# Vandermode/ELD

Measured on AMD Instinct MI355X. Metric: raw megapixels/sec (noise-synth + U-Net step), higher is better.
Workload: dtype f32; 1 GPU; BASELINE.json configs[1]: full ELD noise model (PGRU, SonyA7S2 params) on 4x1424x2128 packed raw + U-Net fp32 train step (fwd, L1, bwd, Adam), 8 frames per GPU; images_per_gpu=8, global_batch=8, parallelism=dp1

## Files before the change

eld_amd/csrc/conv_wgrad.hip:

```cpp
#include <stdlib.h>
#include "conv.h"

#define TW 32
#define JB 32

typedef __bf16 bf16x8 __attribute__((ext_vector_type(8)));
typedef short s16x4 __attribute__((ext_vector_type(4)));
typedef int i32x4_t __attribute__((ext_vector_type(4)));
typedef _Float16 half8 __attribute__((ext_vector_type(8)));

enum { ALG_F32 = 0, ALG_BFM = 1, ALG_X3 = 2, ALG_H2 = 3 };

template <typename T, int MODE, int WCO, int TH, int ALG>
__global__ __launch_bounds__(256, 2) void wgrad_kernel(const WgradArgs a) {
    constexpr bool BFM = ALG == ALG_BFM, X3 = ALG == ALG_X3, H2 = ALG == ALG_H2;
    static_assert(!(X3 || H2) || sizeof(T) == 4, "x3 / h2: fp32 inputs");
    constexpr int ES = sizeof(T);
    constexpr int EPU = 16 / ES;
    constexpr int LES = X3 ? 6 : (BFM ? 2 : 4);
    constexpr int TAPS = MODE == CONV_3X3 ? 9 : 4;
    constexpr int WPIX = 4 / WCO;
    constexpr int COB = 32 * WCO;
    constexpr int TPIX = TH * TW;
    constexpr int PW = TPIX / WPIX;
// ... 237 lines not shown
        for (int s_ = 0; s_ < KS; ++s_) {
            const int cur = s_ & 1;
            if (s_ + 1 < KS) read_step(s_ + 1, fa[cur ^ 1], fb[cur ^ 1]);
            __builtin_amdgcn_sched_barrier(0);
            bsum += fa[cur];
#pragma unroll
            for (int t = 0; t < TAPS; ++t) acc[t] = __builtin_amdgcn_mfma_f32_32x32x2f32(fa[cur], fb[cur][t], acc[t], 0, 0, 0);
            __builtin_amdgcn_sched_barrier(0);
        }
        }
    }

    __syncthreads();
    float* red = lds;
    const size_t pbase = (size_t)ps * TAPS * a.CA * a.CBp;
#pragma unroll
    for (int t = 0; t < TAPS; ++t) {
        if (WPIX > 1) {
            if (wpix > 0) {
#pragma unroll
                for (int i = 0; i < 16; ++i) red[(((wpix - 1) * WCO + wco) * 16 + i) * 64 + lane] = acc[t][i];
            }
            __syncthreads();
            if (wpix == 0) {
                for (int w = 0; w < WPIX - 1; ++w)
#pragma unroll
                    for (int i = 0; i < 16; ++i) acc[t][i] += red[((w * WCO + wco) * 16 + i) * 64 + lane];
            }
            __syncthreads();
        }
        if (wpix == 0) {
#pragma unroll
            for (int i = 0; i < 16; ++i) {
                const int row = (i & 3) + 8 * (i >> 2) + 4 * hi;
                a.part[pbase + ((size_t)t * a.CA + i0 + wco * 32 + row) * a.CBp + j0 + m] = H2 ? acc[t][i] * (1.0f / sc_g) * (1.0f / sc_x) : acc[t][i];
            }
        }
    }
    if (a.bpart && jb == 0) {
        red[wave * 64 + lane] = bsum;
        __syncthreads();
        if (tid < COB) {
            const int wc = tid / 32, mm = tid % 32;
            float s = 0.f;
            for (int wp = 0; wp < WPIX; ++wp) s += red[(wp * WCO + wc) * 64 + mm] + red[(wp * WCO + wc) * 64 + 32 + mm];
            a.bpart[(size_t)ps * a.CA + i0 + tid] = H2 ? s * (1.0f / sc_g) : s;
        }
    }
    if constexpr (XSUM) {
        if (xsum_on) {
            __syncthreads();
            float* r = lds;
#pragma unroll
            for (int e = 0; e < EPU; ++e) r[tid * EPU + e] = xs[e];
            __syncthreads();
            if (tid < JB) {
                constexpr int PARTS = JB / EPU;
                const int part = tid / EPU, comp = tid % EPU;
                float s = 0.f;
                for (int k = 0; k < 256 / PARTS; ++k) s += r[(k * PARTS + part) * EPU + comp];
                a.xbpart[(size_t)ps * a.CBp + j0 + tid] = s;
            }
        }
    }
}

template <typename T, int WCO, int WCI, int WPIX, int TH, int TWT, int STREAM = 0>
__global__ __launch_bounds__(512, 2) void wgrad8_kernel(const WgradArgs a) {
    constexpr int ES = sizeof(T), EPU = 16 / ES, NPC = ES == 4 ? 3 : 1, XQ = 32 / EPU;
    static_assert(WCO * WCI * WPIX == 8, "8 waves");
    constexpr int THREADS = 512, TAPS = 9;
    constexpr int COB = 32 * WCO, JBK = 32 * WCI, TPIX = TH * TWT, PW = TPIX / WPIX, KSB = PW / 16;
    static_assert(TWT == 8 || TWT == 16 || TWT == 32, "tile width");
    static_assert(PW % 16 == 0 && PW >= 16, "a wave's pixel slice is a whole number of 16-pixel k-steps");
    constexpr int X_PIX = (TH + 2) * (TWT + 2);
    constexpr int GBLK = TPIX * 32 + (ES == 4 ? 32 : 0);
    constexpr int GPL = GBLK * WCO, XPL = X_PIX * JBK;
    constexpr int G_Q = COB / EPU, G_UNITS = TPIX * G_Q, G_IT = G_UNITS / THREADS;
    static_assert(G_UNITS % THREADS == 0 && THREADS % G_Q == 0, "a thread stages the same channel quad of G in every iteration");
    constexpr int X_UNITS1 = X_PIX * XQ, X_IT = (X_UNITS1 + THREADS - 1) / THREADS;
    extern __shared__ __attribute__((aligned(16))) float lds[];
    bf16_t* ldsG = reinterpret_cast<bf16_t*>(lds);
    bf16_t* ldsX = ldsG + NPC * GPL;

    const int tid = threadIdx.x, lane = tid & 63, wave = tid >> 6;
    const int m = lane & 31, hi = lane >> 5;
    const int wco = wave % WCO, wci = (wave / WCO) % WCI, wpix = wave / (WCO * WCI);
    const int IB = a.CA / COB, JBn = a.CBp / JBK;
    int bid = xcd_block(a.xcd);
    const int jb = bid % JBn; bid /= JBn;
    const int ib = bid % IB;
    const int ps = bid / IB;
    const int i0 = ib * COB, j0 = jb * JBK;
    const bool do_bias = a.bpart != nullptr && jb == 0;

    f32x16 acc[TAPS];
#pragma unroll
    for (int t = 0; t < TAPS; ++t)
#pragma unroll
        for (int i = 0; i < 16; ++i) acc[t][i] = 0.f;
    float4 bsum4 = make_float4(0.f, 0.f, 0.f, 0.f), bsum4b = make_float4(0.f, 0.f, 0.f, 0.f);

    const int ntiles = a.tiles_x * a.tiles_y;
    const int VP = a.vp;
    const bool seam = VP % TH != 0;
    constexpr unsigned OOB = 0xFFFFFFF0u;
    constexpr int G_STEP = THREADS / G_Q;
    const int g_part = tid % G_Q, g_lp0 = tid / G_Q;
    const int g_px0 = g_lp0 % TWT, g_py0 = g_lp0 / TWT;
    const unsigned g_off0 = (unsigned)(g_px0 * a.CA + i0 + g_part * EPU) * (unsigned)ES;
    const int g_lds0 = ((g_part * EPU) >> 5) * GBLK + g_lp0 * 32 + ((g_part * EPU) & 31);
    auto g_pxy = [&](int it, int& dpx, int& dpy) {
        if (G_STEP >= TWT) { dpx = 0; dpy = it * (G_STEP / TWT); }
        else { dpx = (it * G_STEP) % TWT; dpy = (it * G_STEP) / TWT; }
    };
    const int x_part = (int)((unsigned)tid % (unsigned)XQ);
    int x_hyx[X_IT];
#pragma unroll
    for (int it = 0; it < X_IT; ++it) {
        const int hp = (int)((unsigned)(tid + it * THREADS) / (unsigned)XQ);
        const int hy = hp / (TWT + 2);
        x_hyx[it] = (hy << 8) | (hp - hy * (TWT + 2));
    }
    auto x_alive = [&](int it) { return (it + 1) * THREADS <= X_UNITS1 || (int)((unsigned)(tid + it * THREADS) / (unsigned)XQ) < X_PIX; };
    const char* xs[WCI]; int xC[WCI], xc0[WCI];
#pragma unroll
    for (int cb = 0; cb < WCI; ++cb) {
        const int c = j0 + cb * 32;
        if (c < a.C0) { xs[cb] = static_cast<const char*>(a.x0); xC[cb] = a.C0; xc0[cb] = c; }
        else if (c < a.C0 + a.C1) { xs[cb] = static_cast<const char*>(a.x1); xC[cb] = a.C1; xc0[cb] = c - a.C0; }
        else { xs[cb] = nullptr; xC[cb] = 32; xc0[cb] = 0; }
    }
    float4 rg[G_IT], rx[WCI][X_IT];
    const size_t g_img = (size_t)a.H * a.W * a.CA * ES;
    const unsigned g_rowc = (unsigned)(g_py0 * a.W * a.CA) * (unsigned)ES;
    auto load_tile = [&](int tile) {
        int ty, tx;
        band_tile(tile, a.tiles_x, a.tiles_y, a.band, ty, tx);
        const int v0 = ty * TH, x0 = tx * TWT;
        const int img0 = v0 / VP, vrel = v0 - img0 * VP;
        const int wrem = a.W - x0;
        if (!seam || VP - vrel > TH) {
            const __amdgpu_buffer_rsrc_t rs_g = __builtin_amdgcn_make_buffer_rsrc((void*)(static_cast<const char*>(a.g) + (size_t)img0 * g_img), 0, (int)g_img, 0x00020000);
            const int gbase = (vrel * a.W + x0) * a.CA * ES;
#pragma unroll
            for (int it = 0; it < G_IT; ++it) {
                int dpx, dpy;
                g_pxy(it, dpx, dpy);
                const unsigned off = g_off0 + g_rowc + (unsigned)((dpy * a.W + dpx) * a.CA) * (unsigned)ES;
                rg[it] = __builtin_bit_cast(float4, __builtin_amdgcn_raw_buffer_load_b128(rs_g, g_px0 + dpx < wrem ? (int)off : (int)OOB, gbase, 0));
            }
#pragma unroll
            for (int cb = 0; cb < WCI; ++cb) {
                const size_t x_img = (size_t)a.H * a.W * xC[cb] * ES;
                const __amdgpu_buffer_rsrc_t rs_x = __builtin_amdgcn_make_buffer_rsrc((void*)(xs[cb] ? xs[cb] + (size_t)img0 * x_img : nullptr), 0, xs[cb] ? (int)x_img : 0, 0x00020000);
#pragma unroll
                for (int it = 0; it < X_IT; ++it) {
                    const int gy = vrel - 1 + (x_hyx[it] >> 8), gx = x0 - 1 + (x_hyx[it] & 255);
                    const bool ok = x_alive(it) && (unsigned)gy < (unsigned)a.H && (unsigned)gx < (unsigned)a.W;
                    const unsigned off = ok ? (unsigned)((gy * a.W + gx) * xC[cb] + xc0[cb] + x_part * EPU) * (unsigned)ES : OOB;
                    rx[cb][it] = __builtin_bit_cast(float4, __builtin_amdgcn_raw_buffer_load_b128(rs_x, (int)off, 0, 0));
                }
            }
            return;
        }
        const int nimg = a.N - img0 < 2 ? a.N - img0 : 2;
        const int lim0 = a.H - vrel, nxt = VP - vrel;
        const __amdgpu_buffer_rsrc_t rs_g = __builtin_amdgcn_make_buffer_rsrc((void*)(static_cast<const char*>(a.g) + (size_t)img0 * g_img), 0, (int)(g_img * nimg), 0x00020000);
        const unsigned gb0 = (unsigned)((vrel * a.W + x0) * a.CA) * (unsigned)ES;
        const unsigned gb1 = (unsigned)(((a.H - nxt) * a.W + x0) * a.CA) * (unsigned)ES;
#pragma unroll
        for (int it = 0; it < G_IT; ++it) {
            int dpx, dpy;
            g_pxy(it, dpx, dpy);
            const int r = g_py0 + dpy;
            const bool second = r >= nxt;
            const bool ok = (r < lim0 || (second && r - nxt < a.H)) && g_px0 + dpx < wrem;
            const unsigned off = (second ? gb1 : gb0) + g_off0 + g_rowc + (unsigned)((dpy * a.W + dpx) * a.CA) * (unsigned)ES;
            rg[it] = __builtin_bit_cast(float4, __builtin_amdgcn_raw_buffer_load_b128(rs_g, ok ? (int)off : (int)OOB, 0, 0));
        }
#pragma unroll
        for (int cb = 0; cb < WCI; ++cb) {
            const size_t x_img = (size_t)a.H * a.W * xC[cb] * ES;
            const __amdgpu_buffer_rsrc_t rs_x = __builtin_amdgcn_make_buffer_rsrc((void*)(xs[cb] ? xs[cb] + (size_t)img0 * x_img : nullptr), 0, xs[cb] ? (int)(x_img * nimg) : 0, 0x00020000);
#pragma unroll
            for (int it = 0; it < X_IT; ++it) {
                const int r = (x_hyx[it] >> 8) - 1, gx = x0 - 1 + (x_hyx[it] & 255);
                const bool second = r >= nxt;
                const int wrow = second ? a.H + r - nxt : vrel + r;
                const bool rok = second ? r - nxt < a.H : (unsigned)(vrel + r) < (unsigned)a.H;
                const bool ok = x_alive(it) && rok && (unsigned)gx < (unsigned)a.W;
                const unsigned off = ok ? (unsigned)((wrow * a.W + gx) * xC[cb] + xc0[cb] + x_part * EPU) * (unsigned)ES : OOB;
                rx[cb][it] = __builtin_bit_cast(float4, __builtin_amdgcn_raw_buffer_load_b128(rs_x, (int)off, 0, 0));
            }
        }
    };
    auto put3 = [&](bf16_t* d, int plane_elems, const float4& raw) {
        if constexpr (ES == 2) { *reinterpret_cast<float4*>(d) = raw; return; }
        const unsigned x0 = __float_as_uint(raw.x), x1 = __float_as_uint(raw.y), x2 = __float_as_uint(raw.z), x3 = __float_as_uint(raw.w);
        const float r0 = raw.x - __uint_as_float(x0 & 0xFFFF0000u), r1 = raw.y - __uint_as_float(x1 & 0xFFFF0000u);
        const float r2 = raw.z - __uint_as_float(x2 & 0xFFFF0000u), r3 = raw.w - __uint_as_float(x3 & 0xFFFF0000u);
        const unsigned y0 = __float_as_uint(r0), y1 = __float_as_uint(r1), y2 = __float_as_uint(r2), y3 = __float_as_uint(r3);
        const unsigned z0 = __float_as_uint(r0 - __uint_as_float(y0 & 0xFFFF0000u)), z1 = __float_as_uint(r1 - __uint_as_float(y1 & 0xFFFF0000u));
        const unsigned z2 = __float_as_uint(r2 - __uint_as_float(y2 & 0xFFFF0000u)), z3 = __float_as_uint(r3 - __uint_as_float(y3 & 0xFFFF0000u));
        auto hp = [](unsigned lo, unsigned hi_) { return __builtin_amdgcn_perm(hi_, lo, 0x07060302u); };
        *reinterpret_cast<uint2*>(d) = make_uint2(hp(x0, x1), hp(x2, x3));
        *reinterpret_cast<uint2*>(d + plane_elems) = make_uint2(hp(y0, y1), hp(y2, y3));
        *reinterpret_cast<uint2*>(d + 2 * plane_elems) = make_uint2(hp(z0, z1), hp(z2, z3));
    };
    auto store_tile = [&]() {
#pragma unroll
        for (int it = 0; it < G_IT; ++it) {
            put3(ldsG + g_lds0 + it * G_STEP * 32, GPL, rg[it]);
            if (do_bias) {
                if constexpr (ES == 4) { bsum4.x += rg[it].x; bsum4.y += rg[it].y; bsum4.z += rg[it].z; bsum4.w += rg[it].w; }
                else {
                    const uint4 q = __builtin_bit_cast(uint4, rg[it]);
                    const float4 lo = unpack_bf4(make_uint2(q.x, q.y)), hi4 = unpack_bf4(make_uint2(q.z, q.w));
                    bsum4.x += lo.x; bsum4.y += lo.y; bsum4.z += lo.z; bsum4.w += lo.w;
                    bsum4b.x += hi4.x; bsum4b.y += hi4.y; bsum4b.z += hi4.z; bsum4b.w += hi4.w;
                }
            }
        }
#pragma unroll
        for (int cb = 0; cb < WCI; ++cb)
#pragma unroll
            for (int it = 0; it < X_IT; ++it)
                if (x_alive(it)) put3(ldsX + (cb * X_PIX + (int)((unsigned)(tid + it * THREADS) / (unsigned)XQ)) * 32 + x_part * EPU, XPL, rx[cb][it]);
    };

    const int gi = lane & 15, gg = lane >> 4;
    constexpr bool ROWSHARE = STREAM == 2;
    static_assert(!ROWSHARE || (NPC == 3 && TWT == 8 && WPIX == 1 && TH % 2 == 0), "row-shared fragments: fp32, 8-pixel-wide tiles, one pixel slice");
    constexpr int HS = TH / 2;
    const int lq0 = ROWSHARE ? HS * TWT * hi + (gi >> 2) : wpix * PW + 8 * hi + (gi >> 2);
    const int pyq = lq0 / TWT, pxq = lq0 - pyq * TWT;
    const bf16_t* gq = ldsG + wco * GBLK + lq0 * 32 + (gg & 1) * 16 + (gi & 3) * 4;
    const bf16_t* xq = ldsX + (wci * X_PIX + pyq * (TWT + 2) + pxq) * 32 + (gg & 1) * 16 + (gi & 3) * 4;
    auto tr8 = [](const bf16_t* p0) {
        const s16x4 lo = __builtin_amdgcn_ds_read_tr16_b64_v4i16((__attribute__((address_space(3))) s16x4*)p0);
        const s16x4 hi4 = __builtin_amdgcn_ds_read_tr16_b64_v4i16((__attribute__((address_space(3))) s16x4*)(p0 + 4 * 32));
        return __builtin_bit_cast(bf16x8, __builtin_shufflevector(lo, hi4, 0, 1, 2, 3, 4, 5, 6, 7));
    };

    if (ps < ntiles) load_tile(ps);
    for (int tile = ps; tile < ntiles; tile += a.psplit) {
        __syncthreads();
        store_tile();
        __syncthreads();
        if (tile + a.psplit < ntiles) load_tile(tile + a.psplit);
        if constexpr (ROWSHARE) {
            constexpr int GI[6] = {0, 1, 2, 0, 1, 0};
            constexpr int XI[6] = {2, 1, 0, 1, 0, 0};
            constexpr int NU = (HS + 2) * 3;
            bf16x8 gr[3][3], xf[2][3];
            auto readG = [&](int s_, bf16x8 (&g3)[3]) {
#pragma unroll
                for (int pc = 0; pc < 3; ++pc) g3[pc] = tr8(gq + pc * GPL + s_ * TWT * 32);
            };
            auto readF = [&](int a_, int kx, bf16x8 (&x3)[3]) {
#pragma unroll
                for (int pc = 0; pc < 3; ++pc) x3[pc] = tr8(xq + pc * XPL + (a_ * (TWT + 2) + kx) * 32);
            };
            readG(0, gr[0]);
            readF(0, 0, xf[0]);
#pragma unroll
            for (int u = 0; u < NU; ++u) {
                const int a_ = u / 3, kx = u % 3;
                if (u + 1 < NU) readF((u + 1) / 3, (u + 1) % 3, xf[(u + 1) & 1]);
                __builtin_amdgcn_sched_barrier(0);
#pragma unroll
                for (int ky = 2; ky >= 0; --ky) {
                    const int s_ = a_ - ky;
                    if (s_ >= 0 && s_ < HS) {
#pragma unroll
                        for (int q = 0; q < 6; ++q)
                            acc[3 * ky + kx] = __builtin_amdgcn_mfma_f32_32x32x16_bf16(gr[s_ % 3][GI[q]], xf[u & 1][XI[q]], acc[3 * ky + kx], 0, 0, 0);
                    }
                    if (ky == 2 && kx == 2 && a_ + 1 < HS) {
                        __builtin_amdgcn_sched_barrier(0);
                        readG(a_ + 1, gr[(a_ + 1) % 3]);
                    }
                }
                __builtin_amdgcn_sched_barrier(0);
            }
        } else
        if constexpr (NPC == 3 && STREAM == 1) {
            constexpr int GI[6] = {0, 1, 2, 0, 1, 0};
            constexpr int XI[6] = {2, 1, 0, 1, 0, 0};
            constexpr int NBLK = KSB * TAPS;
            bf16x8 ga[2][3], xb[2][3];
            auto readG = [&](int ks, bf16x8 (&g3)[3]) {
#pragma unroll
                for (int pc = 0; pc < 3; ++pc) g3[pc] = tr8(gq + pc * GPL + ks * 16 * 32);
            };
            auto readX = [&](int ks, int t, bf16x8 (&x3)[3]) {
                const int lrel = ks * 16, dy0 = lrel / TWT, dxp = lrel - dy0 * TWT;
                const int xoff = (dy0 + t / 3) * (TWT + 2) + dxp + t % 3;
#pragma unroll
                for (int pc = 0; pc < 3; ++pc) x3[pc] = tr8(xq + pc * XPL + xoff * 32);
            };
            readG(0, ga[0]);
            readX(0, 0, xb[0]);
#pragma unroll
            for (int b = 0; b < NBLK; ++b) {
                const int ks = b / TAPS, t = b % TAPS;
                if (b + 1 < NBLK) {
                    const int ks1 = (b + 1) / TAPS, t1 = (b + 1) % TAPS;
                    readX(ks1, t1, xb[(b + 1) & 1]);
                    if (ks1 != ks) readG(ks1, ga[ks1 & 1]);
                }
                __builtin_amdgcn_sched_barrier(0);
#pragma unroll
                for (int q = 0; q < 6; ++q) acc[t] = __builtin_amdgcn_mfma_f32_32x32x16_bf16(ga[ks & 1][GI[q]], xb[b & 1][XI[q]], acc[t], 0, 0, 0);
                __builtin_amdgcn_sched_barrier(0);
            }
        } else
#pragma unroll
        for (int ks = 0; ks < KSB; ++ks) {
            const int lrel = ks * 16;
            const int dy0 = lrel / TWT, dxp = lrel - dy0 * TWT;
            bf16x8 ga[NPC];
#pragma unroll
            for (int pc = 0; pc < NPC; ++pc) ga[pc] = tr8(gq + pc * GPL + lrel * 32);
#pragma unroll
            for (int t0 = 0; t0 < TAPS; t0 += 3) {
                bf16x8 xb[3][NPC];
#pragma unroll
                for (int tt = 0; tt < 3; ++tt) {
                    const int xoff = (dy0 + t0 / 3) * (TWT + 2) + dxp + tt;
#pragma unroll
                    for (int pc = 0; pc < NPC; ++pc) xb[tt][pc] = tr8(xq + pc * XPL + xoff * 32);
                }
                if constexpr (NPC == 3) {
                    constexpr int GI[6] = {0, 1, 2, 0, 1, 0};
                    constexpr int XI[6] = {2, 1, 0, 1, 0, 0};
#pragma unroll
                    for (int q = 0; q < 6; ++q)
#pragma unroll
                        for (int tt = 0; tt < 3; ++tt)
                            acc[t0 + tt] = __builtin_amdgcn_mfma_f32_32x32x16_bf16(ga[GI[q]], xb[tt][XI[q]], acc[t0 + tt], 0, 0, 0);
                } else {
#pragma unroll
                    for (int tt = 0; tt < 3; ++tt) acc[t0 + tt] = __builtin_amdgcn_mfma_f32_32x32x16_bf16(ga[0], xb[tt][0], acc[t0 + tt], 0, 0, 0);
                }
                __builtin_amdgcn_sched_barrier(0);
            }
        }
    }

    __syncthreads();
    float* red = lds;
    const size_t pbase = (size_t)ps * TAPS * a.CA * a.CBp;
    const int wt = wci * WCO + wco;
#pragma unroll
    for (int t = 0; t < TAPS; ++t) {
        if (WPIX > 1) {
            if (wpix > 0) {
#pragma unroll
                for (int i = 0; i < 16; ++i) red[(((wpix - 1) * (WCO * WCI) + wt) * 16 + i) * 64 + lane] = acc[t][i];
            }
            __syncthreads();
            if (wpix == 0) {
                for (int w = 0; w < WPIX - 1; ++w)
#pragma unroll
                    for (int i = 0; i < 16; ++i) acc[t][i] += red[((w * (WCO * WCI) + wt) * 16 + i) * 64 + lane];
            }
            __syncthreads();
        }
        if (wpix == 0) {
#pragma unroll
            for (int i = 0; i < 16; ++i) {
                const int row = (i & 3) + 8 * (i >> 2) + 4 * hi;
                a.part[pbase + ((size_t)t * a.CA + i0 + wco * 32 + row) * a.CBp + j0 + wci * 32 + m] = acc[t][i];
            }
        }
    }
    if (do_bias) {
        __syncthreads();
        if constexpr (ES == 4) reinterpret_cast<float4*>(red)[tid] = bsum4;
        else { reinterpret_cast<float4*>(red)[2 * tid] = bsum4; reinterpret_cast<float4*>(red)[2 * tid + 1] = bsum4b; }
        __syncthreads();
        if (tid < COB) {
            const int q = tid / EPU, comp = tid % EPU;
            float s_ = 0.f;
            for (int k = 0; k < THREADS / G_Q; ++k) s_ += red[(q + k * G_Q) * EPU + comp];
            a.bpart[(size_t)ps * a.CA + i0 + tid] = s_;
        }
    }
}

__device__ __forceinline__ void wg_dma16(i32x4_t rsrc, unsigned voff, unsigned lds_dst) {
    unsigned keep;
    asm volatile("s_nop 4\n\ts_mov_b32 %0, m0\n\ts_mov_b32 m0, %3\n\ts_nop 0\n\tbuffer_load_dwordx4 %1, %2, 0 offen lds\n\ts_mov_b32 m0, %0"
                 : "=&s"(keep) : "v"(voff), "s"(rsrc), "s"(lds_dst) : "memory");
}

template <int WCO, int WCI, int WPIX, int TH, int TWT>
__global__ __launch_bounds__(512, 2) void wgrad8d_kernel(const WgradArgs a) {
    static_assert(WCO * WCI * WPIX == 8, "8 waves");
    static_assert(TWT == 8 || TWT == 16 || TWT == 32, "tile width");
    constexpr int WAVES = 8, THREADS = 512, TAPS = 9;
    constexpr int COB = 32 * WCO, JBK = 32 * WCI, TPIX = TH * TWT, PW = TPIX / WPIX, KSB = PW / 16;
    static_assert(PW % 16 == 0 && PW >= 16, "a wave's pixel slice is a whole number of 16-pixel k-steps");
    constexpr int HW = TWT + 2, X_PIX = (TH + 2) * HW;
    static_assert((TPIX * 4) % 64 == 0, "a block of G is whole DMA pieces");
    constexpr int GB_PIECES = TPIX * 4 / 64, XB_PIECES = (X_PIX * 4 + 63) / 64;
    constexpr int G_PIECES = WCO * GB_PIECES, X_PIECES = WCI * XB_PIECES;
    constexpr int G_IT = (G_PIECES + WAVES - 1) / WAVES, X_IT = (X_PIECES + WAVES - 1) / WAVES;
    constexpr int GBLK = GB_PIECES * 512, XBLK = XB_PIECES * 512;
    constexpr int BUF_BYTES = (G_PIECES + X_PIECES) * 1024;
    extern __shared__ __attribute__((aligned(16))) float lds[];

    const int tid = threadIdx.x, lane = tid & 63;
    const int wave = __builtin_amdgcn_readfirstlane(tid >> 6);
    const int m = lane & 31, hi = lane >> 5;
    const int wco = wave % WCO, wci = (wave / WCO) % WCI, wpix = wave / (WCO * WCI);
    const int IB = a.CA / COB, JBn = a.CBp / JBK;
    int bid = xcd_block(a.xcd);
    const int jb = bid % JBn; bid /= JBn;
    const int ib = bid % IB;
    const int ps = bid / IB;
    const int i0 = ib * COB, j0 = jb * JBK;
    const bool do_bias = a.bpart != nullptr && jb == 0;

    f32x16 acc[TAPS];
#pragma unroll
    for (int t = 0; t < TAPS; ++t)
#pragma unroll
        for (int i = 0; i < 16; ++i) acc[t][i] = 0.f;
// ... 96 lines not shown
    static_assert(TPIX % B_STEP == 0, "bias pass covers the tile");
    const int g_part = tid % G_Q;
    const bf16_t* bq0 = ldsG + (g_part >> 2) * GBLK + (tid / G_Q) * 32 + (g_part & 3) * 8;

    int buf = 0;
    if (ps < ntiles) issue(ps, 0);
    for (int tile = ps; tile < ntiles; tile += a.psplit) {
        asm volatile("s_waitcnt vmcnt(0)" ::: "memory");
        __syncthreads();
        if (tile + a.psplit < ntiles) issue(tile + a.psplit, buf ^ 1);
        const int bo = buf * (BUF_BYTES / 2);
        if (do_bias) {
#pragma unroll
            for (int k = 0; k < B_IT; ++k) {
                const uint4 q = *reinterpret_cast<const uint4*>(bq0 + bo + k * B_STEP * 32);
                const float4 lo = unpack_bf4(make_uint2(q.x, q.y)), hi4 = unpack_bf4(make_uint2(q.z, q.w));
                bsum4.x += lo.x; bsum4.y += lo.y; bsum4.z += lo.z; bsum4.w += lo.w;
                bsum4b.x += hi4.x; bsum4b.y += hi4.y; bsum4b.z += hi4.z; bsum4b.w += hi4.w;
            }
        }
        const bf16_t* gq = gq0 + bo;
        const bf16_t* xq = xq0 + bo;
#pragma unroll
        for (int ks = 0; ks < KSB; ++ks) {
            const int lrel = ks * 16;
            const int dy0 = lrel / TWT, dxp = lrel - dy0 * TWT;
            const bf16x8 ga = tr8(gq + lrel * 32);
#pragma unroll
            for (int t0 = 0; t0 < TAPS; t0 += 3) {
                bf16x8 xb[3];
#pragma unroll
                for (int tt = 0; tt < 3; ++tt) xb[tt] = tr8(xq + ((dy0 + t0 / 3) * HW + dxp + tt) * 32);
#pragma unroll
                for (int tt = 0; tt < 3; ++tt) acc[t0 + tt] = __builtin_amdgcn_mfma_f32_32x32x16_bf16(ga, xb[tt], acc[t0 + tt], 0, 0, 0);
            }
        }
        buf ^= 1;
    }

    __syncthreads();
    float* red = lds;
    const size_t pbase = (size_t)ps * TAPS * a.CA * a.CBp;
    const int wt = wci * WCO + wco;
#pragma unroll
    for (int t = 0; t < TAPS; ++t) {
        if (WPIX > 1) {
            if (wpix > 0) {
#pragma unroll
                for (int i = 0; i < 16; ++i) red[(((wpix - 1) * (WCO * WCI) + wt) * 16 + i) * 64 + lane] = acc[t][i];
            }
            __syncthreads();
            if (wpix == 0) {
                for (int w = 0; w < WPIX - 1; ++w)
#pragma unroll
                    for (int i = 0; i < 16; ++i) acc[t][i] += red[((w * (WCO * WCI) + wt) * 16 + i) * 64 + lane];
            }
            __syncthreads();
        }
        if (wpix == 0) {
#pragma unroll
            for (int i = 0; i < 16; ++i) {
                const int row = (i & 3) + 8 * (i >> 2) + 4 * hi;
                a.part[pbase + ((size_t)t * a.CA + i0 + wco * 32 + row) * a.CBp + j0 + wci * 32 + m] = acc[t][i];
            }
        }
    }
    if (do_bias) {
        __syncthreads();
        reinterpret_cast<float4*>(red)[2 * tid] = bsum4; reinterpret_cast<float4*>(red)[2 * tid + 1] = bsum4b;
        __syncthreads();
        if (tid < COB) {
            const int q = tid / 8, comp = tid % 8;
            float s_ = 0.f;
            for (int k = 0; k < THREADS / G_Q; ++k) s_ += red[(q + k * G_Q) * 8 + comp];
            a.bpart[(size_t)ps * a.CA + i0 + tid] = s_;
        }
    }
}

static int wgrad8_dma() {
    static const int on = [] { const char* e = getenv("ELD_WGRAD_DMA"); return e ? (int)(atoi(e) != 0) : 1; }();
    return on && !(debug_kernel_mask(-1) & 16);
}
template <int DUMMY>
__global__ __launch_bounds__(512, 2) void wgradt8_kernel(const WgradArgs a) {
    constexpr int WCO = 4, WCI = 2, TH = 8, TWT = 8, TPIX = TH * TWT, THREADS = 512, TAPS = 4, NPC = 3;
    constexpr int COB = 32 * WCO, JBK = 32 * WCI, KSB = TPIX / 16;
    constexpr int GBLK = TPIX * 32 + 32;
    constexpr int GPL = GBLK * WCO, X_PIX = TAPS * TPIX, XPL = X_PIX * JBK;
    constexpr int G_IT = TPIX * (COB / 4) / THREADS, X_IT = X_PIX * 8 / THREADS;
    extern __shared__ __attribute__((aligned(16))) float lds[];
    bf16_t* ldsG = reinterpret_cast<bf16_t*>(lds);
    bf16_t* ldsX = ldsG + NPC * GPL;
    const int tid = threadIdx.x, lane = tid & 63, wave = tid >> 6;
    const int m = lane & 31, hi = lane >> 5;
    const int wco = wave % WCO, wci = wave / WCO;
    const int IB = a.CA / COB, JBn = a.CBp / JBK;
    int bid = xcd_block(a.xcd);
    const int jb = bid % JBn; bid /= JBn;
    const int ib = bid % IB;
    const int ps = bid / IB;
    const int i0 = ib * COB, j0 = jb * JBK;
    const bool xsum_on = a.xbpart != nullptr && ib == 0;
    const int Wx = 2 * a.W, CB = a.C0;

    f32x16 acc[TAPS];
#pragma unroll
    for (int t = 0; t < TAPS; ++t)
#pragma unroll
        for (int i = 0; i < 16; ++i) acc[t][i] = 0.f;
    float4 xs4[WCI];
#pragma unroll
    for (int cb = 0; cb < WCI; ++cb) xs4[cb] = make_float4(0.f, 0.f, 0.f, 0.f);

    const int tiles_per_img = a.tiles_x * a.tiles_y, ntiles = tiles_per_img * a.N;
    constexpr unsigned OOB = 0xFFFFFFF0u;
    const int g_part = tid & 31, g_lp0 = tid >> 5, x_part = tid & 7, x_lp = tid >> 3;
    const int x_py = x_lp / TWT, x_px = x_lp - x_py * TWT;
    float4 rg[G_IT], rx[WCI][X_IT];
    const size_t g_img = (size_t)a.H * a.W * a.CA * 4, x_img = (size_t)4 * a.H * a.W * CB * 4;
    auto load_tile = [&](int tile) {
        const int img = tile / tiles_per_img;
        int ty, tx;
        band_tile(tile - img * tiles_per_img, a.tiles_x, a.tiles_y, a.band, ty, tx);
        const int y0 = ty * TH, x0 = tx * TWT;
        const __amdgpu_buffer_rsrc_t rs_g = __builtin_amdgcn_make_buffer_rsrc((void*)(static_cast<const char*>(a.g) + (size_t)img * g_img), 0, (int)g_img, 0x00020000);
        const __amdgpu_buffer_rsrc_t rs_x = __builtin_amdgcn_make_buffer_rsrc((void*)(static_cast<const char*>(a.x0) + (size_t)img * x_img), 0, (int)x_img, 0x00020000);
#pragma unroll
        for (int it = 0; it < G_IT; ++it) {
            const int lp = g_lp0 + 16 * it, py = lp / TWT, px = lp - py * TWT;
            const int gy = y0 + py, gx = x0 + px;
            const unsigned off = (gy < a.H && gx < a.W) ? (unsigned)(((gy * a.W + gx) * a.CA + i0 + g_part * 4) * 4) : OOB;
            rg[it] = __builtin_bit_cast(float4, __builtin_amdgcn_raw_buffer_load_b128(rs_g, (int)off, 0, 0));
        }
        const bool pok = y0 + x_py < a.H && x0 + x_px < a.W;
#pragma unroll
        for (int cb = 0; cb < WCI; ++cb)
#pragma unroll
            for (int it = 0; it < X_IT; ++it) {
                const int gy = 2 * (y0 + x_py) + (it >> 1), gx = 2 * (x0 + x_px) + (it & 1);
                const unsigned off = pok ? (unsigned)(((gy * Wx + gx) * CB + j0 + cb * 32 + x_part * 4) * 4) : OOB;
                rx[cb][it] = __builtin_bit_cast(float4, __builtin_amdgcn_raw_buffer_load_b128(rs_x, (int)off, 0, 0));
            }
    };
    auto put3 = [&](bf16_t* d, int plane_elems, const float4& raw) {
        const unsigned x0 = __float_as_uint(raw.x), x1 = __float_as_uint(raw.y), x2 = __float_as_uint(raw.z), x3 = __float_as_uint(raw.w);
        const float r0 = raw.x - __uint_as_float(x0 & 0xFFFF0000u), r1 = raw.y - __uint_as_float(x1 & 0xFFFF0000u);
        const float r2 = raw.z - __uint_as_float(x2 & 0xFFFF0000u), r3 = raw.w - __uint_as_float(x3 & 0xFFFF0000u);
        const unsigned y0 = __float_as_uint(r0), y1 = __float_as_uint(r1), y2 = __float_as_uint(r2), y3 = __float_as_uint(r3);
        const unsigned z0 = __float_as_uint(r0 - __uint_as_float(y0 & 0xFFFF0000u)), z1 = __float_as_uint(r1 - __uint_as_float(y1 & 0xFFFF0000u));
        const unsigned z2 = __float_as_uint(r2 - __uint_as_float(y2 & 0xFFFF0000u)), z3 = __float_as_uint(r3 - __uint_as_float(y3 & 0xFFFF0000u));
        auto hp = [](unsigned lo, unsigned hi_) { return __builtin_amdgcn_perm(hi_, lo, 0x07060302u); };
        *reinterpret_cast<uint2*>(d) = make_uint2(hp(x0, x1), hp(x2, x3));
        *reinterpret_cast<uint2*>(d + plane_elems) = make_uint2(hp(y0, y1), hp(y2, y3));
        *reinterpret_cast<uint2*>(d + 2 * plane_elems) = make_uint2(hp(z0, z1), hp(z2, z3));
    };
    auto store_tile = [&]() {
#pragma unroll
        for (int it = 0; it < G_IT; ++it)
            put3(ldsG + ((g_part * 4) >> 5) * GBLK + (g_lp0 + 16 * it) * 32 + ((g_part * 4) & 31), GPL, rg[it]);
#pragma unroll
        for (int cb = 0; cb < WCI; ++cb)
#pragma unroll
            for (int it = 0; it < X_IT; ++it) {
                put3(ldsX + (cb * X_PIX + it * TPIX + x_lp) * 32 + x_part * 4, XPL, rx[cb][it]);
                if (xsum_on) { xs4[cb].x += rx[cb][it].x; xs4[cb].y += rx[cb][it].y; xs4[cb].z += rx[cb][it].z; xs4[cb].w += rx[cb][it].w; }
// ... 15 lines not shown
        store_tile();
        __syncthreads();
        if (tile + a.psplit < ntiles) load_tile(tile + a.psplit);
#pragma unroll
        for (int ks = 0; ks < KSB; ++ks) {
            bf16x8 ga[NPC];
#pragma unroll
            for (int pc = 0; pc < NPC; ++pc) ga[pc] = tr8(gq + pc * GPL + ks * 16 * 32);
#pragma unroll
            for (int t0 = 0; t0 < TAPS; t0 += 2) {
                bf16x8 xb[2][NPC];
#pragma unroll
                for (int tt = 0; tt < 2; ++tt)
#pragma unroll
                    for (int pc = 0; pc < NPC; ++pc) xb[tt][pc] = tr8(xq + pc * XPL + ((t0 + tt) * TPIX + ks * 16) * 32);
                constexpr int GI[6] = {0, 1, 2, 0, 1, 0};
                constexpr int XI[6] = {2, 1, 0, 1, 0, 0};
#pragma unroll
                for (int q = 0; q < 6; ++q)
#pragma unroll
                    for (int tt = 0; tt < 2; ++tt)
                        acc[t0 + tt] = __builtin_amdgcn_mfma_f32_32x32x16_bf16(ga[GI[q]], xb[tt][XI[q]], acc[t0 + tt], 0, 0, 0);
            }
        }
    }
    const size_t pbase = (size_t)ps * TAPS * a.CA * a.CBp;
#pragma unroll
    for (int t = 0; t < TAPS; ++t)
#pragma unroll
        for (int i = 0; i < 16; ++i) {
            const int row = (i & 3) + 8 * (i >> 2) + 4 * hi;
            a.part[pbase + ((size_t)t * a.CA + i0 + wco * 32 + row) * a.CBp + j0 + wci * 32 + m] = acc[t][i];
        }
    if (xsum_on) {
        __syncthreads();
        float4* r = reinterpret_cast<float4*>(lds);
#pragma unroll
        for (int cb = 0; cb < WCI; ++cb) r[cb * THREADS + tid] = xs4[cb];
        __syncthreads();
        if (tid < JBK) {
            const int cb = tid >> 5, c = tid & 31, quad = c >> 2, comp = c & 3;
            float s_ = 0.f;
            for (int k = 0; k < THREADS / 8; ++k) s_ += reinterpret_cast<const float*>(&r[cb * THREADS + quad + 8 * k])[comp];
            a.xbpart[(size_t)ps * a.CBp + j0 + tid] = s_;
        }
    }
}

bool wgradt8_takes(int CA, int CB) {
    static const int on = [] { const char* e = getenv("ELD_WGRADT8"); return e ? atoi(e) : 1; }();
    return on && CA % 128 == 0 && CB % 64 == 0;
}
int wgradt8_ntiles(int N, int H, int W) { return ((W + 7) / 8) * ((H + 7) / 8) * N; }

static int launch_wt8(WgradArgs a, hipStream_t st) {
    eld_note_conv_kernel("wgradt8");
    a.xcd = eld_xcd_mask() & XCD_WGRAD8;
    a.band = eld_tile_band();
    a.tiles_x = (a.W + 7) / 8;
    a.tiles_y = (a.H + 7) / 8;
    const size_t lds_bytes = (size_t)(3 * 4 * (64 * 32 + 32) + 3 * 2 * 256 * 32) * 2;
    const long long blocks = (long long)(a.CA / 128) * (a.CBp / 64) * a.psplit;
    if (blocks <= 0) return 0;
    if ((size_t)4 * a.H * a.W * a.C0 * 4 >= 0xFFFFFFF0ull || (size_t)a.H * a.W * a.CA * 4 >= 0xFFFFFFF0ull) return ELD_ENOTSUP;
    auto kern = wgradt8_kernel<0>;
    static EldAttrOnce once;
    { const int rc = once.ensure(kern, lds_bytes); if (rc) return rc; }
    ELD_LAUNCH(kern, dim3((unsigned)blocks), dim3(512), lds_bytes, st, a);
    ELD_LAUNCH_CHECK();
    return 0;
}

bool wgrad8_shape(int CA, int CBp, int& COB, int& JBK, int& TH, int& TWo, bool bf16) {
    if (CA % 32 || CBp % 32) return false;
    TWo = 32;
    if (CA % 128 == 0 && CBp % 64 == 0) { COB = 128; JBK = 64; TH = 2; }
    else if (CA % 64 == 0 && CBp % 64 == 0) { COB = 64; JBK = 64; TH = 2; }
    else if (CA % 64 == 0) { COB = 64; JBK = 32; TH = 4; }
    else if (CBp % 64 == 0) { COB = 32; JBK = 64; TH = 4; }
    else { COB = 32; JBK = 32; TH = 4; }
    if (bf16) TH = 8;
    if (bf16 && wgrad8_dma() && COB == 128) { TH = 16; TWo = 8; return true; }
    if (COB == 128) { TH = TH * 4; TWo = 8; }
    return true;
}

int wgrad8_ntiles(int CA, int CBp, int N, int H, int W, bool bf16) {
    int COB, JBK, TH, TWo;
    if (!wgrad8_shape(CA, CBp, COB, JBK, TH, TWo, bf16)) return 0;
    const int VP = vrow_pitch(N, H, TH);
    return ((W + TWo - 1) / TWo) * ((vrow_extent(N, H, VP) + TH - 1) / TH);
}

template <typename T, int WCO, int WCI, int WPIX, int TH, int TWT, int STREAM = 0>
static int launch_w8(WgradArgs a, hipStream_t st) {
    a.xcd = eld_xcd_mask() & XCD_WGRAD8;
    a.band = eld_tile_band();
    constexpr int COB = 32 * WCO, JBK = 32 * WCI;
    eld_note_conv_variant(sizeof(T) == 2 ? "wgrad8<bf16>" : (COB == 128 ? "wgrad8<f32,128x64>" : (COB == 64 ? (JBK == 64 ? "wgrad8<f32,64x64>" : "wgrad8<f32,64x32>")
                                                                                                     : (JBK == 64 ? "wgrad8<f32,32x64>" : "wgrad8<f32,32x32>"))),
                          STREAM == 1 ? "stream" : (STREAM == 2 ? "rowshare" : nullptr));
    a.vp = vrow_pitch(a.N, a.H, TH);
    a.tiles_x = (a.W + TWT - 1) / TWT;
    a.tiles_y = (vrow_extent(a.N, a.H, a.vp) + TH - 1) / TH;
    size_t lds_bytes = (size_t)((TH * TWT * 32 + (sizeof(T) == 4 ? 32 : 0)) * (COB / 32) + (TH + 2) * (TWT + 2) * JBK) * (sizeof(T) == 4 ? 6 : 2);
    const size_t red_bytes = (size_t)7 * 16 * 64 * sizeof(float) * 1;
    if (lds_bytes < red_bytes) lds_bytes = red_bytes;
    const long long blocks = (long long)(a.CA / COB) * (a.CBp / JBK) * a.psplit;
    if (blocks <= 0) return 0;
    auto kern = wgrad8_kernel<T, WCO, WCI, WPIX, TH, TWT, STREAM>;
    static EldAttrOnce once;
    { const int rc = once.ensure(kern, lds_bytes); if (rc) return rc; }
    ELD_LAUNCH(kern, dim3((unsigned)blocks), dim3(512), lds_bytes, st, a);
    ELD_LAUNCH_CHECK();
    return 0;
}

template <int WCO, int WCI, int WPIX, int TH, int TWT>
static int launch_w8d(WgradArgs a, hipStream_t st) {
    eld_note_conv_kernel("wgrad8d");
    a.xcd = eld_xcd_mask() & XCD_WGRAD8;
    a.band = eld_tile_band();
    constexpr int COB = 32 * WCO, JBK = 32 * WCI;
    a.vp = vrow_pitch(a.N, a.H, TH);
    a.tiles_x = (a.W + TWT - 1) / TWT;
    a.tiles_y = (vrow_extent(a.N, a.H, a.vp) + TH - 1) / TH;
    constexpr int PIECES = WCO * (TH * TWT * 4 / 64) + WCI * (((TH + 2) * (TWT + 2) * 4 + 63) / 64);
    size_t lds_bytes = (size_t)2 * PIECES * 1024;
    const size_t red_bytes = (size_t)7 * 16 * 64 * sizeof(float);
    if (lds_bytes < red_bytes) lds_bytes = red_bytes;
    const long long blocks = (long long)(a.CA / COB) * (a.CBp / JBK) * a.psplit;
    if (blocks <= 0) return 0;
    auto kern = wgrad8d_kernel<WCO, WCI, WPIX, TH, TWT>;
    static EldAttrOnce once;
    { const int rc = once.ensure(kern, lds_bytes); if (rc) return rc; }
    ELD_LAUNCH(kern, dim3((unsigned)blocks), dim3(512), lds_bytes, st, a);
    ELD_LAUNCH_CHECK();
    return 0;
}

static int launch_wgrad8(const WgradArgs& a, hipStream_t st) {
    const bool bf16 = a.dtype == DT_BF16;
    const size_t es = bf16 ? 2 : 4;
    int COB, JBK, TH, TWo;
    if (!wgrad8_shape(a.CA, a.CBp, COB, JBK, TH, TWo, bf16)) return ELD_ENOTSUP;
    if ((a.C0 % 32) || (a.C1 % 32)) return ELD_ENOTSUP;
    const size_t win = a.N > 1 ? 2 : 1;
    if ((size_t)a.H * a.W * a.CA * es * win >= 0xFFFFFFF0ull || (size_t)a.H * a.W * (a.C0 > a.C1 ? a.C0 : a.C1) * es * win >= 0xFFFFFFF0ull) return ELD_ENOTSUP;
    if (bf16 && wgrad8_dma() && COB == 128) {
        return launch_w8d<4, 2, 1, 16, 8>(a, st);
    }
    if (bf16) {
        if (COB == 128) return launch_w8<bf16_t, 4, 2, 1, 32, 8>(a, st);
        if (COB == 64 && JBK == 64) return launch_w8<bf16_t, 2, 2, 2, 8, 32>(a, st);
        if (COB == 64) return launch_w8<bf16_t, 2, 1, 4, 8, 32>(a, st);
        if (JBK == 64) return launch_w8<bf16_t, 1, 2, 4, 8, 32>(a, st);
        return launch_w8<bf16_t, 1, 1, 8, 8, 32>(a, st);
    }
    static const int stream = [] { const char* e = getenv("ELD_WG8_STREAM"); return e ? atoi(e) : 0; }();
    static const int rowshare = [] { const char* e = getenv("ELD_WG8_ROWSHARE"); return e ? atoi(e) : 0; }();
    if (COB == 128 && rowshare) return launch_w8<float, 4, 2, 1, 8, 8, 2>(a, st);
    if (COB == 128) return (stream & 1) ? launch_w8<float, 4, 2, 1, 8, 8, 1>(a, st) : launch_w8<float, 4, 2, 1, 8, 8>(a, st);
    if (stream & 2) {
        if (COB == 64 && JBK == 64) return launch_w8<float, 2, 2, 2, 2, 32, 1>(a, st);
        if (COB == 64) return launch_w8<float, 2, 1, 4, 4, 32, 1>(a, st);
        if (JBK == 64) return launch_w8<float, 1, 2, 4, 4, 32, 1>(a, st);
        return launch_w8<float, 1, 1, 8, 4, 32, 1>(a, st);
    }
    if (COB == 64 && JBK == 64) return launch_w8<float, 2, 2, 2, 2, 32>(a, st);
    if (COB == 64) return launch_w8<float, 2, 1, 4, 4, 32>(a, st);
    if (JBK == 64) return launch_w8<float, 1, 2, 4, 4, 32>(a, st);
    return launch_w8<float, 1, 1, 8, 4, 32>(a, st);
}

template <typename T, int MODE, int WCO, int TH, int ALG = ALG_F32>
static int launch_w(WgradArgs a, hipStream_t st) {
    eld_note_conv_variant(sizeof(T) == 2 ? (MODE == CONV_3X3 ? "wgrad<bf16>" : "wgrad<bf16,gather>") : (MODE == CONV_3X3 ? "wgrad<f32>" : "wgrad<f32,gather>"),
                          (sizeof(T) == 2 && ALG == ALG_F32) ? "f32mma" : nullptr);
    a.xcd = eld_xcd_mask() & XCD_WGRAD;
    constexpr int COB = 32 * WCO;
    constexpr int X_PIX = MODE == CONV_3X3 ? (TH + 2) * (TW + 2) : 4 * TH * TW;
    a.tiles_x = (a.W + TW - 1) / TW;
    a.tiles_y = (a.H + TH - 1) / TH;
    constexpr int GROWS = TH * TW + ((ALG == ALG_X3 || ALG == ALG_H2) ? 1 : 0);
    size_t lds_bytes = (size_t)(GROWS * COB + X_PIX * JB) * (ALG == ALG_X3 ? 6 : (ALG == ALG_BFM ? 2 : 4));
    const size_t red_bytes = (size_t)4 * 16 * 64 * sizeof(float);
    if (lds_bytes < red_bytes) lds_bytes = red_bytes;
    const long long blocks = (long long)(a.CA / COB) * (a.CBp / JB) * a.psplit;
    if (blocks <= 0) return 0;
    auto kern = wgrad_kernel<T, MODE, WCO, TH, ALG>;
    static EldAttrOnce once;
    { const int rc = once.ensure(kern, lds_bytes); if (rc) return rc; }
    ELD_LAUNCH(kern, dim3((unsigned)blocks), dim3(256), lds_bytes, st, a);
    ELD_LAUNCH_CHECK();
    return 0;
}

int launch_wgrad(const WgradArgs& a, int mode, hipStream_t st) {
    if (a.CA % 32 || a.CBp % 32 || a.C0 % 4 || a.C1 % 4 || a.psplit < 1) return ELD_EINVAL;
    if (a.C1 > 0 && a.C0 % 32) return ELD_EINVAL;
    const bool c64 = a.CA % 64 == 0;
    if (a.dtype == DT_BF16) {
        if (a.C0 % 8 || a.C1 % 8) return ELD_EINVAL;
        if (mode == CONV_3X3 && a.wgrad8) {
            const int rc = launch_wgrad8(a, st);
            if (rc != ELD_ENOTSUP) return rc;
        }
        static const int mma = [] { const char* e = getenv("ELD_WGRAD_BF16_MMA"); return e ? atoi(e) : 1; }();
        if (mma) {
            if (mode == CONV_3X3) return c64 ? launch_w<bf16_t, CONV_3X3, 2, 4, ALG_BFM>(a, st) : launch_w<bf16_t, CONV_3X3, 1, 4, ALG_BFM>(a, st);
            if (mode == CONV_GATHER2X2) return c64 ? launch_w<bf16_t, CONV_GATHER2X2, 2, 2, ALG_BFM>(a, st) : launch_w<bf16_t, CONV_GATHER2X2, 1, 2, ALG_BFM>(a, st);
            return ELD_EINVAL;
        }
        if (mode == CONV_3X3) return c64 ? launch_w<bf16_t, CONV_3X3, 2, 4>(a, st) : launch_w<bf16_t, CONV_3X3, 1, 4>(a, st);
        if (mode == CONV_GATHER2X2) return c64 ? launch_w<bf16_t, CONV_GATHER2X2, 2, 2>(a, st) : launch_w<bf16_t, CONV_GATHER2X2, 1, 2>(a, st);
        return ELD_EINVAL;
    }
    const int algo = resolve_algo(a.algo);
    if (algo == 2) {
        if (!a.amax_g || !a.amax_x0) return ELD_EINVAL;
        if (mode == CONV_3X3) return c64 ? launch_w<float, CONV_3X3, 2, 2, ALG_H2>(a, st) : launch_w<float, CONV_3X3, 1, 4, ALG_H2>(a, st);
        if (mode == CONV_GATHER2X2) return c64 ? launch_w<float, CONV_GATHER2X2, 2, 2, ALG_H2>(a, st) : launch_w<float, CONV_GATHER2X2, 1, 2, ALG_H2>(a, st);
        return ELD_EINVAL;
    }
    if (mode == CONV_3X3 && algo == 1 && a.wgrad8) {
        const int rc = launch_wgrad8(a, st);
        if (rc != ELD_ENOTSUP) return rc;
    }
    if (mode == CONV_3X3 && algo == 1) return c64 ? launch_w<float, CONV_3X3, 2, 2, ALG_X3>(a, st) : launch_w<float, CONV_3X3, 1, 2, ALG_X3>(a, st);
    if (mode == CONV_3X3) return c64 ? launch_w<float, CONV_3X3, 2, 4>(a, st) : launch_w<float, CONV_3X3, 1, 4>(a, st);
    if (mode == CONV_GATHER2X2 && algo == 1 && a.wgrad8 && a.C1 == 0 && a.C0 == a.CBp && wgradt8_takes(a.CA, a.C0)) return launch_wt8(a, st);
    if (mode == CONV_GATHER2X2 && algo == 1) return c64 ? launch_w<float, CONV_GATHER2X2, 2, 2, ALG_X3>(a, st) : launch_w<float, CONV_GATHER2X2, 1, 2, ALG_X3>(a, st);
    if (mode == CONV_GATHER2X2) return c64 ? launch_w<float, CONV_GATHER2X2, 2, 2>(a, st) : launch_w<float, CONV_GATHER2X2, 1, 2>(a, st);
    return ELD_EINVAL;
}

template <int T>
__global__ __launch_bounds__(1024) void wgrad_reduce_kernel(const float* __restrict__ part, const float* __restrict__ bpart, float* __restrict__ wgrad,
                                                            float* __restrict__ bgrad, int psplit, int CA, int CBp, int CBr, int pair_blocks, int NB) {
    extern __shared__ float sh[];
    const int lane = threadIdx.x & 63, w = threadIdx.x >> 6, NW = blockDim.x >> 6;
    const size_t pairs = (size_t)CA * CBp, plane = pairs * T;
    if ((int)blockIdx.x >= pair_blocks) {
        const int c = ((int)blockIdx.x - pair_blocks) * 64 + lane;
        float b = 0.f;
        if (c < NB) {
            int k = w;
            for (; k + 3 * NW < psplit; k += 4 * NW)
                b += (bpart[(size_t)k * NB + c] + bpart[(size_t)(k + NW) * NB + c]) + (bpart[(size_t)(k + 2 * NW) * NB + c] + bpart[(size_t)(k + 3 * NW) * NB + c]);
            for (; k < psplit; k += NW) b += bpart[(size_t)k * NB + c];
// ... 65 lines not shown
```

Before: 701.4 raw MPix/s.

## Double-buffer LDS plane sets in fp32 wgrad8 with split-wave staging

Adds a STREAM==3 variant of the fp32 wgrad8 kernel that keeps two LDS plane sets and alternates between them. While MFMA work reads the current set, half of the waves stage the next tile into the other set before computing and the other half after computing. This leaves one barrier per tile instead of two and overlaps global loads and LDS stores with compute. To fit two sets in LDS, the tile height drops for the 32- and 64-channel non-64x64 shapes, which may reduce reuse per tile. The variant is on by default and can be turned off with a debug mask bit or a stream env setting.

Result: no change. 704.6 raw MPix/s (median of 6 runs) (+0.4%).

```diff
diff --git a/eld_amd/csrc/conv_wgrad.hip b/eld_amd/csrc/conv_wgrad.hip
--- a/eld_amd/csrc/conv_wgrad.hip
+++ b/eld_amd/csrc/conv_wgrad.hip
@@ -343,8 +343,11 @@
     extern __shared__ __attribute__((aligned(16))) float lds[];
     bf16_t* ldsG = reinterpret_cast<bf16_t*>(lds);
     bf16_t* ldsX = ldsG + NPC * GPL;
-
-    const int tid = threadIdx.x, lane = tid & 63, wave = tid >> 6;
+    constexpr bool DPL = STREAM == 3;
+    constexpr int PSET = NPC * (GPL + XPL);
+    static_assert(!DPL || (ES == 4 && 2 * PSET * 2 <= 160 * 1024), "two plane sets fit the CU's LDS");
+
+    const int tid = threadIdx.x, lane = tid & 63, wave = DPL ? __builtin_amdgcn_readfirstlane(tid >> 6) : tid >> 6;
     const int m = lane & 31, hi = lane >> 5;
     const int wco = wave % WCO, wci = (wave / WCO) % WCI, wpix = wave / (WCO * WCI);
     const int IB = a.CA / COB, JBn = a.CBp / JBK;
@@ -469,10 +472,10 @@
         *reinterpret_cast<uint2*>(d + plane_elems) = make_uint2(hp(y0, y1), hp(y2, y3));
         *reinterpret_cast<uint2*>(d + 2 * plane_elems) = make_uint2(hp(z0, z1), hp(z2, z3));
     };
-    auto store_tile = [&]() {
+    auto store_tile = [&](int pset = 0) {
 #pragma unroll
         for (int it = 0; it < G_IT; ++it) {
-            put3(ldsG + g_lds0 + it * G_STEP * 32, GPL, rg[it]);
+            put3(ldsG + pset + g_lds0 + it * G_STEP * 32, GPL, rg[it]);
             if (do_bias) {
                 if constexpr (ES == 4) { bsum4.x += rg[it].x; bsum4.y += rg[it].y; bsum4.z += rg[it].z; bsum4.w += rg[it].w; }
                 else {
@@ -487,7 +490,7 @@
         for (int cb = 0; cb < WCI; ++cb)
 #pragma unroll
             for (int it = 0; it < X_IT; ++it)
-                if (x_alive(it)) put3(ldsX + (cb * X_PIX + (int)((unsigned)(tid + it * THREADS) / (unsigned)XQ)) * 32 + x_part * EPU, XPL, rx[cb][it]);
+                if (x_alive(it)) put3(ldsX + pset + (cb * X_PIX + (int)((unsigned)(tid + it * THREADS) / (unsigned)XQ)) * 32 + x_part * EPU, XPL, rx[cb][it]);
     };
 
     const int gi = lane & 15, gg = lane >> 4;
@@ -496,8 +499,8 @@
     constexpr int HS = TH / 2;
     const int lq0 = ROWSHARE ? HS * TWT * hi + (gi >> 2) : wpix * PW + 8 * hi + (gi >> 2);
     const int pyq = lq0 / TWT, pxq = lq0 - pyq * TWT;
-    const bf16_t* gq = ldsG + wco * GBLK + lq0 * 32 + (gg & 1) * 16 + (gi & 3) * 4;
-    const bf16_t* xq = ldsX + (wci * X_PIX + pyq * (TWT + 2) + pxq) * 32 + (gg & 1) * 16 + (gi & 3) * 4;
+    const bf16_t* gq0 = ldsG + wco * GBLK + lq0 * 32 + (gg & 1) * 16 + (gi & 3) * 4;
+    const bf16_t* xq0 = ldsX + (wci * X_PIX + pyq * (TWT + 2) + pxq) * 32 + (gg & 1) * 16 + (gi & 3) * 4;
     auto tr8 = [](const bf16_t* p0) {
         const s16x4 lo = __builtin_amdgcn_ds_read_tr16_b64_v4i16((__attribute__((address_space(3))) s16x4*)p0);
         const s16x4 hi4 = __builtin_amdgcn_ds_read_tr16_b64_v4i16((__attribute__((address_space(3))) s16x4*)(p0 + 4 * 32));
@@ -505,11 +508,30 @@
     };
 
     if (ps < ntiles) load_tile(ps);
+    if constexpr (DPL) {
+        if (ps < ntiles) store_tile(0);
+        if (ps + a.psplit < ntiles) load_tile(ps + a.psplit);
+        __syncthreads();
+    }
+    const bool cut_first = wave < 4;
+    int cur = 0;
     for (int tile = ps; tile < ntiles; tile += a.psplit) {
-        __syncthreads();
-        store_tile();
-        __syncthreads();
-        if (tile + a.psplit < ntiles) load_tile(tile + a.psplit);
+        auto stage_next = [&]() {
+            if (tile + a.psplit < ntiles) {
+                store_tile(cur ^ PSET);
+                if (tile + 2 * a.psplit < ntiles) load_tile(tile + 2 * a.psplit);
+            }
+        };
+        if constexpr (DPL) {
+            if (cut_first) stage_next();
+        } else {
+            __syncthreads();
+            store_tile();
+            __syncthreads();
+            if (tile + a.psplit < ntiles) load_tile(tile + a.psplit);
+        }
+        const bf16_t* gq = gq0 + cur;
+        const bf16_t* xq = xq0 + cur;
         if constexpr (ROWSHARE) {
             constexpr int GI[6] = {0, 1, 2, 0, 1, 0};
             constexpr int XI[6] = {2, 1, 0, 1, 0, 0};
@@ -607,6 +629,11 @@
                 }
                 __builtin_amdgcn_sched_barrier(0);
             }
+        }
+        if constexpr (DPL) {
+            if (!cut_first) stage_next();
+            __syncthreads();
+            cur ^= PSET;
         }
     }
 
@@ -869,6 +896,11 @@
     static const int on = [] { const char* e = getenv("ELD_WGRAD_DMA"); return e ? (int)(atoi(e) != 0) : 1; }();
     return on && !(debug_kernel_mask(-1) & 16);
 }
+static int wgrad8_stream() {
+    static const int stream = [] { const char* e = getenv("ELD_WG8_STREAM"); return e ? atoi(e) : 0; }();
+    return stream;
+}
+static bool wgrad8_two_sets() { return !(debug_kernel_mask(-1) & 512) && !(wgrad8_stream() & 2); }
 template <int DUMMY>
 __global__ __launch_bounds__(512, 2) void wgradt8_kernel(const WgradArgs a) {
     constexpr int WCO = 4, WCI = 2, TH = 8, TWT = 8, TPIX = TH * TWT, THREADS = 512, TAPS = 4, NPC = 3;
@@ -1050,6 +1082,7 @@
     if (bf16) TH = 8;
     if (bf16 && wgrad8_dma() && COB == 128) { TH = 16; TWo = 8; return true; }
     if (COB == 128) { TH = TH * 4; TWo = 8; }
+    else if (!bf16 && wgrad8_two_sets() && !(COB == 64 && JBK == 64)) TH = (COB == 32 && JBK == 32) ? 4 : 2;
     return true;
 }
 
@@ -1067,11 +1100,13 @@
     constexpr int COB = 32 * WCO, JBK = 32 * WCI;
     eld_note_conv_variant(sizeof(T) == 2 ? "wgrad8<bf16>" : (COB == 128 ? "wgrad8<f32,128x64>" : (COB == 64 ? (JBK == 64 ? "wgrad8<f32,64x64>" : "wgrad8<f32,64x32>")
                                                                                                      : (JBK == 64 ? "wgrad8<f32,32x64>" : "wgrad8<f32,32x32>"))),
-                          STREAM == 1 ? "stream" : (STREAM == 2 ? "rowshare" : nullptr));
+                          STREAM == 1 ? "stream" : (STREAM == 2 ? "rowshare" : nullptr),
+                          (sizeof(T) == 4 && COB != 128 && !(COB == 64 && JBK == 64) && STREAM == 0) ? "1set" : nullptr);
     a.vp = vrow_pitch(a.N, a.H, TH);
     a.tiles_x = (a.W + TWT - 1) / TWT;
     a.tiles_y = (vrow_extent(a.N, a.H, a.vp) + TH - 1) / TH;
     size_t lds_bytes = (size_t)((TH * TWT * 32 + (sizeof(T) == 4 ? 32 : 0)) * (COB / 32) + (TH + 2) * (TWT + 2) * JBK) * (sizeof(T) == 4 ? 6 : 2);
+    if (STREAM == 3) lds_bytes *= 2;
     const size_t red_bytes = (size_t)7 * 16 * 64 * sizeof(float) * 1;
     if (lds_bytes < red_bytes) lds_bytes = red_bytes;
     const long long blocks = (long long)(a.CA / COB) * (a.CBp / JBK) * a.psplit;
@@ -1125,7 +1160,7 @@
         if (JBK == 64) return launch_w8<bf16_t, 1, 2, 4, 8, 32>(a, st);
         return launch_w8<bf16_t, 1, 1, 8, 8, 32>(a, st);
     }
-    static const int stream = [] { const char* e = getenv("ELD_WG8_STREAM"); return e ? atoi(e) : 0; }();
+    const int stream = wgrad8_stream();
     static const int rowshare = [] { const char* e = getenv("ELD_WG8_ROWSHARE"); return e ? atoi(e) : 0; }();
     if (COB == 128 && rowshare) return launch_w8<float, 4, 2, 1, 8, 8, 2>(a, st);
     if (COB == 128) return (stream & 1) ? launch_w8<float, 4, 2, 1, 8, 8, 1>(a, st) : launch_w8<float, 4, 2, 1, 8, 8>(a, st);
@@ -1134,6 +1169,11 @@
         if (COB == 64) return launch_w8<float, 2, 1, 4, 4, 32, 1>(a, st);
         if (JBK == 64) return launch_w8<float, 1, 2, 4, 4, 32, 1>(a, st);
         return launch_w8<float, 1, 1, 8, 4, 32, 1>(a, st);
+    }
+    if (wgrad8_two_sets() && !(COB == 64 && JBK == 64)) {
+        if (COB == 64) return launch_w8<float, 2, 1, 4, 2, 32, 3>(a, st);
+        if (JBK == 64) return launch_w8<float, 1, 2, 4, 2, 32, 3>(a, st);
+        return launch_w8<float, 1, 1, 8, 4, 32, 3>(a, st);
     }
     if (COB == 64 && JBK == 64) return launch_w8<float, 2, 2, 2, 2, 32>(a, st);
     if (COB == 64) return launch_w8<float, 2, 1, 4, 4, 32>(a, st);
```
